# tjqansthd/GDN-Pytorch

Measured on AMD Instinct MI355X. Metric: training images/sec at 128x416 batch=20, higher is better.
Workload: dtype f32; 1 GPU; DtoD training step (fwd + losses + bwd + fused Adam), batch 20 per GPU, 128x416, fp32, BASELINE configs[1]; global_batch=20, parallelism=dp1, launch=eager, x3=True

## Files before the change

### gdn-pytorch_amd/csrc/gemm_x3.h

```cpp
#pragma once
#include "common.h"

#define X3_TILE 128
#define X3_BK 32

typedef __bf16 x3_bf16x8 __attribute__((ext_vector_type(8)));

__host__ __device__ static inline int x3_sw(int row) { return ((((row >> 1) ^ (row >> 4)) & 1) << 1) | ((row >> 2) & 1); }
__host__ __device__ static inline size_t x3_off(int row, int k, int p, int KB) {
    const int t = row >> 7, r = row & 127, kb = k >> 5, ch = ((k >> 3) & 3) ^ x3_sw(r);
    return ((((size_t)t * KB + kb) * 3 + p) * 128 + r) * 64 + ch * 16 + (k & 7) * 2;
}
__host__ __device__ static inline size_t x3_packed_bytes(int rows, int K) {
    return (size_t)((rows + X3_TILE - 1) / X3_TILE) * (K / X3_BK) * 3 * 128 * 64;
}

__device__ __forceinline__ unsigned x3_cvt2(float lo, float hi) {
    typedef float x3_f2 __attribute__((ext_vector_type(2)));
    typedef __bf16 x3_b2 __attribute__((ext_vector_type(2)));
    const x3_f2 v = {lo, hi};
    return __builtin_bit_cast(unsigned, __builtin_convertvector(v, x3_b2));
}
__device__ __forceinline__ void x3_split2(float x, float y, unsigned& p1, unsigned& p2, unsigned& p3) {
    p1 = x3_cvt2(x, y);
    const float rx = x - __uint_as_float(p1 << 16), ry = y - __uint_as_float(p1 & 0xffff0000u);
    p2 = x3_cvt2(rx, ry);
    const float sx = rx - __uint_as_float(p2 << 16), sy = ry - __uint_as_float(p2 & 0xffff0000u);
    p3 = x3_cvt2(sx, sy);
}

void launch_gemm_x3_nt(const float* A, const void* Bp, float* C, int bins, int M, int N, int K, hipStream_t st);
#define X3_NT_AUTO GDN_X3_NT_AUTO
#define X3_NT_ONESHOT_128 GDN_X3_NT_ONESHOT_128
#define X3_NT_ONESHOT_64 GDN_X3_NT_ONESHOT_64
#define X3_NT_UNITS_128 GDN_X3_NT_UNITS_128
#define X3_NT_UNITS_64 GDN_X3_NT_UNITS_64
#define X3_NT_KEEP_BINS GDN_X3_NT_KEEP_BINS
#define X3_NT_NO_HALVES GDN_X3_NT_NO_HALVES
#define X3_NT_SHARED GDN_X3_NT_SHARED
void launch_gemm_x3_nt_cfg(const float* A, const void* Bp, float* C, int bins, int M, int N, int K, int cfg, int grid, hipStream_t st);
#define X3_UNITS_PAIRS 1
#define X3_UNITS_HALVE 2
void launch_x3_pack_rows(const float* src, void* dst, int bins, int rows, int K, hipStream_t st);
static inline bool gemm_x3_ok(int M, int N, int K) { return M >= 1 && N >= 128 && N % 128 == 0 && K >= 32 && K % 32 == 0; }
void launch_gemm_x3_tn(const float* A, const float* Bm, float* P, int bins, int T, int NI, int NJ, int nsplit, hipStream_t st);
static inline bool gemm_x3_tn_ok(int T, int NI, int NJ) { return T >= 1 && NI >= 128 && NI % 128 == 0 && NJ >= 128 && NJ % 128 == 0; }
static inline int gemm_x3_tn_splits(int bins, int T, int NI, int NJ) {
    const int wgs = (NI / 128) * (NJ / 128) * bins;
    int best = 1;
    double best_c = 1e30;
    for (int s = 1; s <= 16; ++s) {
        if (s > 1 && T / s < 256) break;
        const double c = (double)((wgs * s + 511) / 512) / s +
                         0.23 * (s - 1) * (1040.0 / T) * ((double)bins * NI * NJ / (36.0 * 512 * 512));
        if (c < best_c - 1e-9) { best_c = c; best = s; }
    }
    return best;
}
```

### gdn-pytorch_amd/csrc/gemm_x3.hip

```cpp
#include "gemm_x3.h"


namespace {

__global__ __launch_bounds__(256) void x3_pack_rows_kernel(const float* __restrict__ src, unsigned char* __restrict__ dst, int rows,
                                                           int K, int rows_pad) {
    const int KB = K / X3_BK, k8n = K / 8;
    const int bin = blockIdx.y;
    const size_t per_bin = x3_packed_bytes(rows, K);
    for (int64_t i = blockIdx.x * 256ll + threadIdx.x; i < (int64_t)rows_pad * k8n; i += (int64_t)gridDim.x * 256) {
        const int row = (int)((i >> 2) % rows_pad), k8 = (int)(i & 3) + 4 * (int)((i >> 2) / rows_pad);
        f32x4 lo = {0.f, 0.f, 0.f, 0.f}, hi = lo;
        if (row < rows) {
            const float* s = src + ((size_t)bin * rows + row) * K + k8 * 8;
            lo = *reinterpret_cast<const f32x4*>(s);
            hi = *reinterpret_cast<const f32x4*>(s + 4);
        }
        unsigned h[3][4];
        x3_split2(lo[0], lo[1], h[0][0], h[1][0], h[2][0]);
        x3_split2(lo[2], lo[3], h[0][1], h[1][1], h[2][1]);
        x3_split2(hi[0], hi[1], h[0][2], h[1][2], h[2][2]);
        x3_split2(hi[2], hi[3], h[0][3], h[1][3], h[2][3]);
#pragma unroll
        for (int p = 0; p < 3; ++p) {
            const uint4 v = {h[p][0], h[p][1], h[p][2], h[p][3]};
            *reinterpret_cast<uint4*>(dst + (size_t)bin * per_bin + x3_off(row, k8 * 8, p, KB)) = v;
        }
    }
}

template <bool DYN = false>
__device__ __forceinline__ void x3_stage_mfma(const unsigned char* As, const unsigned char* Bs, int a_base, int b_base, int h, int f_sw,
                                              f32x16 (&acc)[2][2], f32x16 (&cor)[2][2], int ni = 2) {
#pragma unroll
    for (int s = 0; s < 2; ++s) {
        const int co = ((2 * s + h) ^ f_sw) * 16;
        x3_bf16x8 af[2][3], bf[2][3];
#pragma unroll
        for (int i = 0; i < 2; ++i)
#pragma unroll
            for (int p = 0; p < 3; ++p) {
                af[i][p] = __builtin_bit_cast(x3_bf16x8, *reinterpret_cast<const uint4*>(&As[p * 8192 + a_base + i * 2048 + co]));
                bf[i][p] = __builtin_bit_cast(x3_bf16x8, *reinterpret_cast<const uint4*>(&Bs[p * 8192 + b_base + i * 2048 + co]));
            }
#pragma unroll
        for (int i = 0; i < 2; ++i) {
            if (DYN && i >= ni) continue;
#pragma unroll
            for (int j = 0; j < 2; ++j) {
                cor[i][j] = __builtin_amdgcn_mfma_f32_32x32x16_bf16(af[i][2], bf[j][0], cor[i][j], 0, 0, 0);
                cor[i][j] = __builtin_amdgcn_mfma_f32_32x32x16_bf16(af[i][1], bf[j][1], cor[i][j], 0, 0, 0);
                cor[i][j] = __builtin_amdgcn_mfma_f32_32x32x16_bf16(af[i][0], bf[j][2], cor[i][j], 0, 0, 0);
                cor[i][j] = __builtin_amdgcn_mfma_f32_32x32x16_bf16(af[i][1], bf[j][0], cor[i][j], 0, 0, 0);
                cor[i][j] = __builtin_amdgcn_mfma_f32_32x32x16_bf16(af[i][0], bf[j][1], cor[i][j], 0, 0, 0);
                acc[i][j] = __builtin_amdgcn_mfma_f32_32x32x16_bf16(af[i][0], bf[j][0], acc[i][j], 0, 0, 0);
            }
        }
    }
}

struct X3Walk { int xcd, slot, G8, NT, MT, p0, pairs, full, halved, n; };
struct X3Unit { int bin, m0, nt, hm; };

template <bool UNITS, int TM>
__device__ __forceinline__ X3Unit x3_unit(const X3Walk& w, int i) {
    X3Unit u;
    int ul = i * w.G8 + w.slot, half = 0;
    u.hm = 0;
    if (UNITS && i >= w.full && w.halved) {
        ul = w.full * w.G8 + (w.slot >> 1);
        half = w.slot & 1;
        u.hm = 1;
    }
    const int pl = ul / w.NT, pg = w.p0 + pl, b = pg / w.MT;
    u.nt = ul - pl * w.NT;
    u.bin = w.pairs ? b : b * 8 + w.xcd;
    u.m0 = (pg - b * w.MT) * TM + half * (TM / 2);
    return u;
}

template <bool UNITS, int TM>
__device__ __forceinline__ X3Walk x3_walk(int M, int N, int bins, int mode) {
    X3Walk w;
    w.xcd = blockIdx.x & 7;
    w.slot = blockIdx.x >> 3;
    w.G8 = UNITS ? (int)(gridDim.x >> 3) : 0;
    w.NT = N / 128;
    w.MT = (M + TM - 1) / TM;
    w.pairs = UNITS && (mode & X3_UNITS_PAIRS);
    w.p0 = 0;
    w.full = 1;
    w.halved = 0;
    if (!UNITS) {
        w.n = (w.slot / (w.NT * w.MT)) * 8 + w.xcd < bins ? 1 : 0;
        return w;
    }
    const int P = bins * w.MT;
    int np = w.xcd < bins ? ((bins - 1 - w.xcd) / 8 + 1) * w.MT : 0;
    if (w.pairs) {
        w.p0 = P * w.xcd / 8;
        np = P * (w.xcd + 1) / 8 - w.p0;
    }
    const int U = np * w.NT;
    w.full = U / w.G8;
    const int R = U - w.full * w.G8;
    w.halved = (mode & X3_UNITS_HALVE) && R > 0 && 2 * R <= w.G8;
    w.n = w.full + (w.slot < (w.halved ? 2 * R : R) ? 1 : 0);
    if (w.halved && w.n > w.full && x3_unit<UNITS, TM>(w, w.full).m0 >= M) --w.n;
    return w;
}

template <bool UNITS>
__global__ __launch_bounds__(256, 2) void gemm_x3_nt_kernel(const float* __restrict__ A, const unsigned char* __restrict__ Bp,
                                                            float* __restrict__ C, int M, int N, int K, int bins, int mode) {
    __shared__ __attribute__((aligned(16))) unsigned char As[3 * 128 * 64], Bs[3 * 128 * 64];
    const int tid = threadIdx.x, lane = tid & 63, wave = __builtin_amdgcn_readfirstlane(tid >> 6), wm = wave >> 1, wn = wave & 1;
    const int KB = K / X3_BK;
    const X3Walk w = x3_walk<UNITS, 128>(M, N, bins, mode);
    if (w.n == 0) return;

    f32x16 acc[2][2], cor[2][2];

    const int k4 = tid & 7, rb0 = tid >> 3;
    const float* ap[4];
    const unsigned char* Bb;
    auto aim = [&](const X3Unit& u) {
        const float* Ab = A + (size_t)u.bin * M * K;
#pragma unroll
        for (int v = 0; v < 4; ++v) {
            const int row = v * 32 + rb0;
            ap[v] = Ab + (size_t)(u.m0 + row < M ? u.m0 + row : M - 1) * K + k4 * 4;
        }
        Bb = Bp + (size_t)u.bin * x3_packed_bytes(N, K) + (size_t)u.nt * KB * (3 * 128 * 64);
    };
    f32x4 ra[4];
    f32x4 rb[6];
    auto gload = [&](int kb) {
#pragma unroll
        for (int v = 0; v < 4; ++v) ra[v] = *reinterpret_cast<const f32x4*>(ap[v] + (size_t)kb * X3_BK);
        const unsigned char* bsrc = Bb + (size_t)kb * (3 * 128 * 64) + tid * 16;
#pragma unroll
        for (int v = 0; v < 6; ++v) rb[v] = *reinterpret_cast<const f32x4*>(bsrc + v * 4096);
    };
    auto lstore = [&]() {
#pragma unroll
        for (int v = 0; v < 4; ++v) {
            const int row = v * 32 + rb0;
            unsigned h0[3], h1[3];
            x3_split2(ra[v][0], ra[v][1], h0[0], h0[1], h0[2]);
            x3_split2(ra[v][2], ra[v][3], h1[0], h1[1], h1[2]);
            const int off = row * 64 + (((k4 >> 1) ^ x3_sw(row)) * 16) + (k4 & 1) * 8;
#pragma unroll
            for (int p = 0; p < 3; ++p) {
                const uint2 w = {h0[p], h1[p]};
                *reinterpret_cast<uint2*>(&As[p * 8192 + off]) = w;
            }
        }
#pragma unroll
        for (int v = 0; v < 6; ++v) *reinterpret_cast<f32x4*>(&Bs[v * 4096 + tid * 16]) = rb[v];
    };
    const int r32 = lane & 31, h = lane >> 5;
    const int f_sw = x3_sw(r32);
    const int b_base = (wn * 64 + r32) * 64;
    auto wave_rows = [&](const X3Unit& u, int& wrow, int& nb) {
        wrow = u.hm ? wm * 32 : wm * 64;
        const int left = (M - u.m0 - wrow + 31) >> 5, most = u.hm ? 1 : 2;
        nb = left < 0 ? 0 : left < most ? left : most;
    };
    auto store = [&](const X3Unit& u, int wrow, int nb) {
        float* Cb = C + (size_t)u.bin * M * N;
#pragma unroll
        for (int i = 0; i < 2; ++i) {
            if (i >= nb) continue;
#pragma unroll
            for (int j = 0; j < 2; ++j) {
                const int col = u.nt * 128 + wn * 64 + j * 32 + r32;
#pragma unroll
                for (int r = 0; r < 16; ++r) {
                    const int m = u.m0 + wrow + i * 32 + (r & 3) + 8 * (r >> 2) + 4 * h;
                    if (m < M) Cb[(size_t)m * N + col] = acc[i][j][r] + cor[i][j][r];
                }
            }
        }
    };

    X3Unit cu = x3_unit<UNITS, 128>(w, 0), pu = cu;
    int wrow, nb, pwrow = 0, pnb = 0;
    aim(cu);
    gload(0);
    for (int u = 0;; ++u) {
        const bool more = UNITS && u + 1 < w.n;
        wave_rows(cu, wrow, nb);
        const int a_base = (wrow + r32) * 64;
        lstore();
        __syncthreads();
        if (UNITS && u > 0) store(pu, pwrow, pnb);
#pragma unroll
        for (int i = 0; i < 2; ++i)
#pragma unroll
            for (int j = 0; j < 2; ++j)
#pragma unroll
                for (int r = 0; r < 16; ++r) { acc[i][j][r] = 0.f; cor[i][j][r] = 0.f; }
        for (int kb = 0; kb < KB; ++kb) {
            if (kb > 0) {
                lstore();
                __syncthreads();
            }
            if (kb + 1 < KB) gload(kb + 1);
            else if (more) {
                aim(x3_unit<UNITS, 128>(w, u + 1));
                gload(0);
            }
            if (nb) x3_stage_mfma<true>(As, Bs, a_base, b_base, h, f_sw, acc, cor, nb);
            __syncthreads();
        }
        if (!more) break;
        pu = cu; pwrow = wrow; pnb = nb;
        cu = x3_unit<UNITS, 128>(w, u + 1);
    }
    store(cu, wrow, nb);
}

template <int TM, bool UNITS>
__global__ __launch_bounds__(512, 2) void gemm_x3_nt8_kernel(const float* __restrict__ A, const unsigned char* __restrict__ Bp,
                                                             float* __restrict__ C, int M, int N, int K, int bins, int mode) {
    constexpr int MI = TM / 64, A_BYTES = 3 * TM * 64, B_BYTES = 3 * 128 * 64;
    __shared__ __attribute__((aligned(16))) unsigned char As[2][A_BYTES], Bs[2][B_BYTES];
    const int tid = threadIdx.x, lane = tid & 63, wave = __builtin_amdgcn_readfirstlane(tid >> 6), wm = wave >> 2, wn = wave & 3;
    const int KB = K / X3_BK;
    const X3Walk w = x3_walk<UNITS, TM>(M, N, bins, mode);
    if (w.n == 0) return;
    f32x16 acc[MI], cor[MI];
    const int k4 = tid & 7, rb0 = tid >> 3;
    const float* ap[MI];
    const unsigned char* Bb;
    auto aim = [&](const X3Unit& u) {
        const float* Ab = A + (size_t)u.bin * M * K;
#pragma unroll
        for (int v = 0; v < MI; ++v) {
            const int row = v * 64 + rb0;
            ap[v] = Ab + (size_t)(u.m0 + row < M ? u.m0 + row : M - 1) * K + k4 * 4;
        }
        Bb = Bp + (size_t)u.bin * x3_packed_bytes(N, K) + (size_t)u.nt * KB * B_BYTES;
    };
    f32x4 ra[MI], rb[3];
    auto gload = [&](int kb) {
#pragma unroll
        for (int v = 0; v < MI; ++v) ra[v] = *reinterpret_cast<const f32x4*>(ap[v] + (size_t)kb * X3_BK);
        const unsigned char* bsrc = Bb + (size_t)kb * B_BYTES + tid * 16;
#pragma unroll
        for (int v = 0; v < 3; ++v) rb[v] = *reinterpret_cast<const f32x4*>(bsrc + v * 8192);
    };
    auto lstore = [&](int buf) {
#pragma unroll
        for (int v = 0; v < MI; ++v) {
            const int row = v * 64 + rb0;
            unsigned h0[3], h1[3];
            x3_split2(ra[v][0], ra[v][1], h0[0], h0[1], h0[2]);
            x3_split2(ra[v][2], ra[v][3], h1[0], h1[1], h1[2]);
            const int off = row * 64 + (((k4 >> 1) ^ x3_sw(row)) * 16) + (k4 & 1) * 8;
#pragma unroll
            for (int p = 0; p < 3; ++p) {
                const uint2 w = {h0[p], h1[p]};
                *reinterpret_cast<uint2*>(&As[buf][p * TM * 64 + off]) = w;
            }
        }
#pragma unroll
        for (int v = 0; v < 3; ++v) *reinterpret_cast<f32x4*>(&Bs[buf][v * 8192 + tid * 16]) = rb[v];
    };
    const int r32 = lane & 31, h = lane >> 5;
    const int f_sw = x3_sw(r32);
    const int wrow = wm * (TM / 2);
    const int a_base = (wrow + r32) * 64, b_base = (wn * 32 + r32) * 64;
    auto wave_rows = [&](const X3Unit& u, int& mend, int& nb) {
        const int top = u.m0 + (u.hm ? TM / 2 : TM);
        mend = top < M ? top : M;
        const int left = (mend - u.m0 - wrow + 31) >> 5;
        nb = left < 0 ? 0 : left < MI ? left : MI;
    };
    auto store = [&](const X3Unit& u, int mend, int nb) {
        float* Cb = C + (size_t)u.bin * M * N;
        const int col = u.nt * 128 + wn * 32 + r32;
#pragma unroll
        for (int i = 0; i < MI; ++i) {
            if (i >= nb) continue;
#pragma unroll
            for (int r = 0; r < 16; ++r) {
                const int m = u.m0 + wrow + i * 32 + (r & 3) + 8 * (r >> 2) + 4 * h;
                if (m < mend) Cb[(size_t)m * N + col] = acc[i][r] + cor[i][r];
            }
        }
    };
    int lu = 0, lk = 0;
    auto fetch = [&]() {
        gload(lk);
        if (++lk == KB) {
            lk = 0;
            ++lu;
            if (UNITS && lu < w.n) aim(x3_unit<UNITS, TM>(w, lu));
        }
    };
    const int S = w.n * KB;
    aim(x3_unit<UNITS, TM>(w, 0));
    fetch();
    lstore(0);
    if (S > 1) fetch();
    __syncthreads();
    X3Unit cu = x3_unit<UNITS, TM>(w, 0), pu = cu;
    int mend, nb, pmend = 0, pnb = 0;
    for (int u = 0, g = 0;; ++u) {
        wave_rows(cu, mend, nb);
        for (int kb = 0; kb < KB; ++kb, ++g) {
            const int cur = g & 1;
            if (g + 1 < S) lstore(cur ^ 1);
            if (kb == 0) {
                if (UNITS && u > 0) store(pu, pmend, pnb);
#pragma unroll
                for (int i = 0; i < MI; ++i)
#pragma unroll
                    for (int r = 0; r < 16; ++r) { acc[i][r] = 0.f; cor[i][r] = 0.f; }
            }
            if (g + 2 < S) fetch();
            if (nb > 0) {
#pragma unroll
                for (int s = 0; s < 2; ++s) {
                    const int co = ((2 * s + h) ^ f_sw) * 16;
                    x3_bf16x8 af[MI][3], bf[3];
#pragma unroll
                    for (int p = 0; p < 3; ++p) {
                        bf[p] = __builtin_bit_cast(x3_bf16x8, *reinterpret_cast<const uint4*>(&Bs[cur][p * 8192 + b_base + co]));
#pragma unroll
                        for (int i = 0; i < MI; ++i)
                            if (MI == 1 || i < nb)
                                af[i][p] = __builtin_bit_cast(x3_bf16x8, *reinterpret_cast<const uint4*>(&As[cur][p * TM * 64 + a_base + i * 2048 + co]));
                    }
#pragma unroll
                    for (int i = 0; i < MI; ++i) {
                        if (MI > 1 && i >= nb) continue;
                        cor[i] = __builtin_amdgcn_mfma_f32_32x32x16_bf16(af[i][2], bf[0], cor[i], 0, 0, 0);
                        cor[i] = __builtin_amdgcn_mfma_f32_32x32x16_bf16(af[i][1], bf[1], cor[i], 0, 0, 0);
                        cor[i] = __builtin_amdgcn_mfma_f32_32x32x16_bf16(af[i][0], bf[2], cor[i], 0, 0, 0);
                        cor[i] = __builtin_amdgcn_mfma_f32_32x32x16_bf16(af[i][1], bf[0], cor[i], 0, 0, 0);
                        cor[i] = __builtin_amdgcn_mfma_f32_32x32x16_bf16(af[i][0], bf[1], cor[i], 0, 0, 0);
                        acc[i] = __builtin_amdgcn_mfma_f32_32x32x16_bf16(af[i][0], bf[0], acc[i], 0, 0, 0);
                    }
                }
            }
            __syncthreads();
        }
        if (!(UNITS && u + 1 < w.n)) break;
        pu = cu; pmend = mend; pnb = nb;
        cu = x3_unit<UNITS, TM>(w, u + 1);
    }
    store(cu, mend, nb);
}

__global__ __launch_bounds__(256, 2) void gemm_x3_tn_kernel(const float* __restrict__ A, const float* __restrict__ Bm,
                                                            float* __restrict__ P, int T, int NI, int NJ, int nsplit, int bins) {
    __shared__ __attribute__((aligned(16))) unsigned char As[3 * 128 * 64], Bs[3 * 128 * 64];
    const int tid = threadIdx.x, lane = tid & 63, wave = tid >> 6, wm = wave >> 1, wn = wave & 1;
    const int TI = NI / 128, TJ = NJ / 128;
    const int xcd = blockIdx.x & 7, sq = blockIdx.x >> 3;
    const int bin = (sq / (TI * TJ * nsplit)) * 8 + xcd;
    if (bin >= bins) return;
    const int split = (sq / (TI * TJ)) % nsplit, i0 = ((sq / TJ) % TI) * 128, j0 = (sq % TJ) * 128;
    const int chunk = ((T + nsplit - 1) / nsplit + 31) / 32 * 32;
    const int tb = split * chunk, te = tb + chunk < T ? tb + chunk : T;
    f32x16 acc[2][2], cor[2][2];
#pragma unroll
    for (int i = 0; i < 2; ++i)
#pragma unroll
        for (int j = 0; j < 2; ++j)
#pragma unroll
            for (int r = 0; r < 16; ++r) { acc[i][j][r] = 0.f; cor[i][j][r] = 0.f; }
    const int t8 = tid >> 6, cp = tid & 63;
    const float* ap = A + ((size_t)bin * T) * NI + i0 + cp;
    const float* bp = Bm + ((size_t)bin * T) * NJ + j0 + cp;
    float ra[2][8], rb[2][8];
    auto gload = [&](int t0) {
#pragma unroll
        for (int e = 0; e < 8; ++e) {
            const int t = t0 + t8 * 8 + e;
            const bool in = t < te;
            const int tc = t < T ? t : T - 1;
            const size_t ta = (size_t)tc * NI, tbo = (size_t)tc * NJ;
#pragma unroll
            for (int c = 0; c < 2; ++c) {
                const float va = ap[ta + c * 64], vb = bp[tbo + c * 64];
                ra[c][e] = in ? va : 0.f;
                rb[c][e] = in ? vb : 0.f;
            }
        }
    };
    auto lstore = [&]() {
#pragma unroll
        for (int c = 0; c < 2; ++c) {
            const int row = cp + c * 64;
            const int off = row * 64 + ((t8 ^ x3_sw(row)) * 16);
            unsigned ha[3][4], hb[3][4];
#pragma unroll
            for (int q = 0; q < 4; ++q) {
                x3_split2(ra[c][2 * q], ra[c][2 * q + 1], ha[0][q], ha[1][q], ha[2][q]);
                x3_split2(rb[c][2 * q], rb[c][2 * q + 1], hb[0][q], hb[1][q], hb[2][q]);
            }
#pragma unroll
            for (int p = 0; p < 3; ++p) {
                const uint4 va = {ha[p][0], ha[p][1], ha[p][2], ha[p][3]}, vb = {hb[p][0], hb[p][1], hb[p][2], hb[p][3]};
                *reinterpret_cast<uint4*>(&As[p * 8192 + off]) = va;
                *reinterpret_cast<uint4*>(&Bs[p * 8192 + off]) = vb;
            }
        }
    };
    const int r32 = lane & 31, h = lane >> 5;
    const int f_sw = x3_sw(r32);
    const int a_base = (wm * 64 + r32) * 64, b_base = (wn * 64 + r32) * 64;
    gload(tb);
    for (int t0 = tb; t0 < te; t0 += 32) {
        lstore();
        __syncthreads();
        if (t0 + 32 < te) gload(t0 + 32);
        x3_stage_mfma(As, Bs, a_base, b_base, h, f_sw, acc, cor);
        __syncthreads();
    }
    float* Pb = P + (((size_t)split * bins + bin) * NI) * NJ;
#pragma unroll
    for (int i = 0; i < 2; ++i)
#pragma unroll
        for (int j = 0; j < 2; ++j) {
            const int col = j0 + wn * 64 + j * 32 + r32;
#pragma unroll
            for (int r = 0; r < 16; ++r) {
                const int row = i0 + wm * 64 + i * 32 + (r & 3) + 8 * (r >> 2) + 4 * h;
                Pb[(size_t)row * NJ + col] = acc[i][j][r] + cor[i][j][r];
            }
        }
}

}

void launch_x3_pack_rows(const float* src, void* dst, int bins, int rows, int K, hipStream_t st) {
    const int rows_pad = (rows + X3_TILE - 1) / X3_TILE * X3_TILE;
    const int64_t n = (int64_t)rows_pad * (K / 8);
    const int64_t nb = cdiv64(n, 256);
    hipLaunchKernelGGL(x3_pack_rows_kernel, dim3((unsigned)(nb < 4096 ? nb : 4096), bins), dim3(256), 0, st, src,
                       (unsigned char*)dst, rows, K, rows_pad);
}

static int x3_units_grid() {
    const int g = 2 * gdn_num_cus() / 8 * 8;
    return g < 8 ? 8 : g;
}

void launch_gemm_x3_nt_cfg(const float* A, const void* Bp, float* C, int bins, int M, int N, int K, int cfg, int grid, hipStream_t st) {
    const int NT = N / 128, MT = (M + 127) / 128, bg = (bins + 7) / 8;
    int kern = cfg & 0xff;
    const int gfull = x3_units_grid();
    if (kern == X3_NT_AUTO) {
        const bool small = (int64_t)MT * NT * bins < 4 * 256;
        const int64_t units = (int64_t)(small ? (M + 63) / 64 : MT) * NT * bins;
        const bool walk = units <= 3 * (int64_t)gfull && !(small && (cfg & X3_NT_SHARED));
        kern = small ? (walk ? X3_NT_UNITS_64 : X3_NT_ONESHOT_64) : (walk ? X3_NT_UNITS_128 : X3_NT_ONESHOT_128);
        if (K / X3_BK < 32) cfg |= X3_NT_NO_HALVES;
    }
    const int mode = (cfg & X3_NT_KEEP_BINS ? 0 : X3_UNITS_PAIRS) | (cfg & X3_NT_NO_HALVES ? 0 : X3_UNITS_HALVE);
    const int g = grid > 0 ? grid : gfull;
    const unsigned char* B = (const unsigned char*)Bp;
    switch (kern) {
    case X3_NT_ONESHOT_128:
        hipLaunchKernelGGL(gemm_x3_nt_kernel<false>, dim3(MT * NT * bg * 8), dim3(256), 0, st, A, B, C, M, N, K, bins, 0);
        break;
    case X3_NT_ONESHOT_64:
        hipLaunchKernelGGL((gemm_x3_nt8_kernel<64, false>), dim3(((M + 63) / 64) * NT * bg * 8), dim3(512), 0, st, A, B, C, M, N, K, bins, 0);
        break;
    case X3_NT_UNITS_128:
        hipLaunchKernelGGL(gemm_x3_nt_kernel<true>, dim3(g), dim3(256), 0, st, A, B, C, M, N, K, bins, mode);
        break;
    default:
        hipLaunchKernelGGL((gemm_x3_nt8_kernel<64, true>), dim3(g), dim3(512), 0, st, A, B, C, M, N, K, bins, mode);
        break;
    }
}

void launch_gemm_x3_nt(const float* A, const void* Bp, float* C, int bins, int M, int N, int K, hipStream_t st) {
    launch_gemm_x3_nt_cfg(A, Bp, C, bins, M, N, K, X3_NT_AUTO, 0, st);
}

void launch_gemm_x3_tn(const float* A, const float* Bm, float* P, int bins, int T, int NI, int NJ, int nsplit, hipStream_t st) {
    const int bg = (bins + 7) / 8;
    hipLaunchKernelGGL(gemm_x3_tn_kernel, dim3((NI / 128) * (NJ / 128) * nsplit * bg * 8), dim3(256), 0, st, A, Bm, P, T, NI, NJ,
                       nsplit, bins);
}

extern "C" size_t gdn_gemm_x3_packed_bytes(int32_t bins, int32_t rows, int32_t K) {
    if (bins < 1 || rows < 1 || K < X3_BK || (K % X3_BK)) return 0;
    return (size_t)bins * x3_packed_bytes(rows, K);
}

extern "C" int gdn_gemm_x3_pack(const float* src, void* dst, int32_t bins, int32_t rows, int32_t K, void* stream) {
    (void)hipGetLastError();
    if (!src || !dst || bins < 1 || rows < 1 || K < X3_BK || (K % X3_BK)) return GDN_ERR_BAD_ARG;
    launch_x3_pack_rows(src, dst, bins, rows, K, (hipStream_t)stream);
    return gdn_launch_status();
}

extern "C" int gdn_gemm_x3_nt(const float* A, const void* Bp, float* C, int32_t bins, int32_t M, int32_t N, int32_t K,
                              void* stream) {
    (void)hipGetLastError();
    if (!A || !Bp || !C || bins < 1) return GDN_ERR_BAD_ARG;
    if (!gemm_x3_ok(M, N, K)) return GDN_ERR_UNSUPPORTED;
    launch_gemm_x3_nt(A, Bp, C, bins, M, N, K, (hipStream_t)stream);
    return gdn_launch_status();
}

extern "C" int gdn_gemm_x3_nt_cfg(const float* A, const void* Bp, float* C, int32_t bins, int32_t M, int32_t N, int32_t K,
                                  int32_t cfg, int32_t grid, void* stream) {
    (void)hipGetLastError();
    if (!A || !Bp || !C || bins < 1) return GDN_ERR_BAD_ARG;
    if ((cfg & 0xff) > X3_NT_UNITS_64 || (cfg & ~(0xff | X3_NT_KEEP_BINS | X3_NT_NO_HALVES | X3_NT_SHARED))) return GDN_ERR_BAD_ARG;
    if ((cfg & X3_NT_SHARED) && (cfg & 0xff) != X3_NT_AUTO) return GDN_ERR_BAD_ARG;
    if (grid < 0 || grid % 8 || grid > 8192) return GDN_ERR_BAD_ARG;
    if (!gemm_x3_ok(M, N, K)) return GDN_ERR_UNSUPPORTED;
    launch_gemm_x3_nt_cfg(A, Bp, C, bins, M, N, K, cfg, grid, (hipStream_t)stream);
    return gdn_launch_status();
}

extern "C" int64_t gdn_gemm_x3_tn_splits(int32_t bins, int32_t T, int32_t NI, int32_t NJ) {
    if (bins < 1 || !gemm_x3_tn_ok(T, NI, NJ)) return 0;
    return gemm_x3_tn_splits(bins, T, NI, NJ);
}

extern "C" int gdn_gemm_x3_tn(const float* A, const float* Bm, float* P, int32_t bins, int32_t T, int32_t NI, int32_t NJ,
                              int32_t nsplit, void* stream) {
    (void)hipGetLastError();
    if (!A || !Bm || !P || bins < 1 || T < 1 || nsplit < 1) return GDN_ERR_BAD_ARG;
    if (!gemm_x3_tn_ok(T, NI, NJ)) return GDN_ERR_UNSUPPORTED;
    launch_gemm_x3_tn(A, Bm, P, bins, T, NI, NJ, nsplit, (hipStream_t)stream);
    return gdn_launch_status();
}
```

Measured before the change: 562.7 images/s.

## Overlap bf16x3 split conversion of next A tile with MFMA stage

Moves the fp32-to-triple-bf16 split of the prefetched A (and, in the TN kernel, half of the operands) out of the LDS store phase. It now runs inside the MFMA loop through a fill callback, so the VALU conversion work interleaves with matrix instructions instead of sitting on the critical path between barriers. An empty asm pin keeps the compiler from sinking the split back. In exchange each thread holds pre-split values in more VGPRs, which risks register pressure and lower occupancy. The loop over i is also reversed so the fill lands mid-stage.

```diff
diff --git a/gdn-pytorch_amd/csrc/gemm_x3.h b/gdn-pytorch_amd/csrc/gemm_x3.h
--- a/gdn-pytorch_amd/csrc/gemm_x3.h
+++ b/gdn-pytorch_amd/csrc/gemm_x3.h
@@ -28,6 +28,7 @@
     const float sx = rx - __uint_as_float(p2 << 16), sy = ry - __uint_as_float(p2 & 0xffff0000u);
     p3 = x3_cvt2(sx, sy);
 }
+__device__ __forceinline__ void x3_pin(unsigned& v) { asm volatile("" : "+v"(v)); }
 
 void launch_gemm_x3_nt(const float* A, const void* Bp, float* C, int bins, int M, int N, int K, hipStream_t st);
 #define X3_NT_AUTO GDN_X3_NT_AUTO
diff --git a/gdn-pytorch_amd/csrc/gemm_x3.hip b/gdn-pytorch_amd/csrc/gemm_x3.hip
--- a/gdn-pytorch_amd/csrc/gemm_x3.hip
+++ b/gdn-pytorch_amd/csrc/gemm_x3.hip
@@ -29,9 +29,10 @@
     }
 }
 
-template <bool DYN = false>
+struct X3NoFill { __device__ __forceinline__ void operator()(int) const {} };
+template <bool DYN = false, class Fill = X3NoFill>
 __device__ __forceinline__ void x3_stage_mfma(const unsigned char* As, const unsigned char* Bs, int a_base, int b_base, int h, int f_sw,
-                                              f32x16 (&acc)[2][2], f32x16 (&cor)[2][2], int ni = 2) {
+                                              f32x16 (&acc)[2][2], f32x16 (&cor)[2][2], int ni = 2, Fill fill = Fill()) {
 #pragma unroll
     for (int s = 0; s < 2; ++s) {
         const int co = ((2 * s + h) ^ f_sw) * 16;
@@ -44,8 +45,9 @@
                 bf[i][p] = __builtin_bit_cast(x3_bf16x8, *reinterpret_cast<const uint4*>(&Bs[p * 8192 + b_base + i * 2048 + co]));
             }
 #pragma unroll
-        for (int i = 0; i < 2; ++i) {
-            if (DYN && i >= ni) continue;
+        for (int i = 1; i >= 0; --i) {
+            if (DYN && i > 0 && i >= ni) continue;
+            if (i == 0) fill(s);
 #pragma unroll
             for (int j = 0; j < 2; ++j) {
                 cor[i][j] = __builtin_amdgcn_mfma_f32_32x32x16_bf16(af[i][2], bf[j][0], cor[i][j], 0, 0, 0);
@@ -142,20 +144,28 @@
 #pragma unroll
         for (int v = 0; v < 6; ++v) rb[v] = *reinterpret_cast<const f32x4*>(bsrc + v * 4096);
     };
-    auto lstore = [&]() {
+    uint2 pa[4][3];
+    const int a_off = rb0 * 64 + (((k4 >> 1) ^ x3_sw(rb0)) * 16) + (k4 & 1) * 8;
+    auto split = [&]() {
 #pragma unroll
         for (int v = 0; v < 4; ++v) {
-            const int row = v * 32 + rb0;
             unsigned h0[3], h1[3];
             x3_split2(ra[v][0], ra[v][1], h0[0], h0[1], h0[2]);
             x3_split2(ra[v][2], ra[v][3], h1[0], h1[1], h1[2]);
-            const int off = row * 64 + (((k4 >> 1) ^ x3_sw(row)) * 16) + (k4 & 1) * 8;
 #pragma unroll
             for (int p = 0; p < 3; ++p) {
-                const uint2 w = {h0[p], h1[p]};
-                *reinterpret_cast<uint2*>(&As[p * 8192 + off]) = w;
-            }
-        }
+                x3_pin(h0[p]);
+                x3_pin(h1[p]);
+                pa[v][p] = uint2{h0[p], h1[p]};
+            }
+        }
+    };
+    auto fill = [&](int s) { if (s) split(); };
+    auto lstore = [&]() {
+#pragma unroll
+        for (int v = 0; v < 4; ++v)
+#pragma unroll
+            for (int p = 0; p < 3; ++p) *reinterpret_cast<uint2*>(&As[p * 8192 + v * 2048 + a_off]) = pa[v][p];
 #pragma unroll
         for (int v = 0; v < 6; ++v) *reinterpret_cast<f32x4*>(&Bs[v * 4096 + tid * 16]) = rb[v];
     };
@@ -188,11 +198,14 @@
     int wrow, nb, pwrow = 0, pnb = 0;
     aim(cu);
     gload(0);
+    bool late = true;
     for (int u = 0;; ++u) {
         const bool more = UNITS && u + 1 < w.n;
         wave_rows(cu, wrow, nb);
         const int a_base = (wrow + r32) * 64;
+        if (late) split();
         lstore();
+        late = nb == 0;
         __syncthreads();
         if (UNITS && u > 0) store(pu, pwrow, pnb);
 #pragma unroll
@@ -203,6 +216,7 @@
                 for (int r = 0; r < 16; ++r) { acc[i][j][r] = 0.f; cor[i][j][r] = 0.f; }
         for (int kb = 0; kb < KB; ++kb) {
             if (kb > 0) {
+                if (late) split();
                 lstore();
                 __syncthreads();
             }
@@ -211,7 +225,7 @@
                 aim(x3_unit<UNITS, 128>(w, u + 1));
                 gload(0);
             }
-            if (nb) x3_stage_mfma<true>(As, Bs, a_base, b_base, h, f_sw, acc, cor, nb);
+            if (nb) x3_stage_mfma<true>(As, Bs, a_base, b_base, h, f_sw, acc, cor, nb, fill);
             __syncthreads();
         }
         if (!more) break;
@@ -392,22 +406,29 @@
             }
         }
     };
+    uint4 pa[2][3];
+    const int l_off = cp * 64 + ((t8 ^ x3_sw(cp)) * 16);
+    auto splitc = [&](int c) {
+        unsigned ha[3][4];
+#pragma unroll
+        for (int q = 0; q < 4; ++q) x3_split2(ra[c][2 * q], ra[c][2 * q + 1], ha[0][q], ha[1][q], ha[2][q]);
+#pragma unroll
+        for (int p = 0; p < 3; ++p) {
+#pragma unroll
+            for (int q = 0; q < 4; ++q) x3_pin(ha[p][q]);
+            pa[c][p] = uint4{ha[p][0], ha[p][1], ha[p][2], ha[p][3]};
+        }
+    };
     auto lstore = [&]() {
 #pragma unroll
         for (int c = 0; c < 2; ++c) {
-            const int row = cp + c * 64;
-            const int off = row * 64 + ((t8 ^ x3_sw(row)) * 16);
-            unsigned ha[3][4], hb[3][4];
-#pragma unroll
-            for (int q = 0; q < 4; ++q) {
-                x3_split2(ra[c][2 * q], ra[c][2 * q + 1], ha[0][q], ha[1][q], ha[2][q]);
-                x3_split2(rb[c][2 * q], rb[c][2 * q + 1], hb[0][q], hb[1][q], hb[2][q]);
-            }
+            unsigned hb[3][4];
+#pragma unroll
+            for (int q = 0; q < 4; ++q) x3_split2(rb[c][2 * q], rb[c][2 * q + 1], hb[0][q], hb[1][q], hb[2][q]);
 #pragma unroll
             for (int p = 0; p < 3; ++p) {
-                const uint4 va = {ha[p][0], ha[p][1], ha[p][2], ha[p][3]}, vb = {hb[p][0], hb[p][1], hb[p][2], hb[p][3]};
-                *reinterpret_cast<uint4*>(&As[p * 8192 + off]) = va;
-                *reinterpret_cast<uint4*>(&Bs[p * 8192 + off]) = vb;
+                *reinterpret_cast<uint4*>(&As[p * 8192 + c * 4096 + l_off]) = pa[c][p];
+                *reinterpret_cast<uint4*>(&Bs[p * 8192 + c * 4096 + l_off]) = uint4{hb[p][0], hb[p][1], hb[p][2], hb[p][3]};
             }
         }
     };
@@ -415,11 +436,13 @@
     const int f_sw = x3_sw(r32);
     const int a_base = (wm * 64 + r32) * 64, b_base = (wn * 64 + r32) * 64;
     gload(tb);
+    splitc(0);
+    splitc(1);
     for (int t0 = tb; t0 < te; t0 += 32) {
         lstore();
         __syncthreads();
         if (t0 + 32 < te) gload(t0 + 32);
-        x3_stage_mfma(As, Bs, a_base, b_base, h, f_sw, acc, cor);
+        x3_stage_mfma<false>(As, Bs, a_base, b_base, h, f_sw, acc, cor, 2, splitc);
         __syncthreads();
     }
     float* Pb = P + (((size_t)split * bins + bin) * NI) * NJ;
```

Result: no change. 562.8 images/s, median of 2 (+0.0%).
